# bruAristimunha/Synthetic-Sleep-EEG-Signal-Generation-using-Latent-Diffusion-Models

Measured on AMD Instinct MI355X. Metric: EEG windows/sec (LDM train step), higher is better.
Workload: dtype bf16; 1 GPU; LDM train step on raw (B,1,3072) windows: frozen AutoencoderKL[32,32,64] encode+sample x scale, add_noise, config_ldm.yaml UNet (30.5M params, latent_channels=1) fwd+bwd, epsilon MSE, Adam lr 1e-4 [BASELINE configs[2]/[3]: per-GPU batch 256 = global 2048 / 8]; per_gpu_batch=256, global_batch=256, latent_len=768, parallelism=dp1

## Files before the change

synthetic-sleep-eeg-signal-generation-using-latent-diffusion-models_amd/csrc/internal.h:

```cpp
#pragma once
#include "common.h"

int ew_temb(eegldm_ctx*, const int64_t* t, void* out, int B, int dim, int dtype);
int ew_silu(eegldm_ctx*, const float* x, void* y, long n, int dtype);
int ew_silu_bwd(eegldm_ctx*, const float* dy, const float* x, void* dx, long n, int dtype);
int eeg_det_buffer(eegldm_ctx*, size_t bytes, float** out);
int ew_fold_partials_det(eegldm_ctx*, const float* parts, int nparts, long stride, int off, int n, float* total);
int ew_colsum(eegldm_ctx*, const void* x, long ldx, float* out_ps, long ldo, float* total, int B, int L, int C, int dtype);
int ew_softmax(eegldm_ctx*, const float* S, void* P, long rows, int n, int dtype);
int ew_softmax_bwd(eegldm_ctx*, const float* dP, const void* P, void* dS, long rows, int n, float alpha, int dtype);
int ew_add_rows(eegldm_ctx*, void* dst, long ldd, const void* src, long lds, long rows, int C, int dtype);
int ew_dropout_rows(eegldm_ctx*, void* x, long ld, long rows, int C, float p, uint64_t seed, uint64_t offset, int dtype);
int ew_film_silu_fwd(eegldm_ctx*, const void* hn, long ldh, const float* emb, long lde, void* a, long lda, int B, int L, int C, int dtype);
int ew_film_silu_bwd(eegldm_ctx*, const void* hn, long ldh, const float* emb, long lde, const void* da, long ldda, void* dhn, long lddh,
                     float* demb, long ldde, int B, int L, int C, int dtype);
int ew_copy_rows(eegldm_ctx*, void* dst, long ldd, const void* src, long lds, long rows, int C, int dtype);
int ew_label_emb_add(eegldm_ctx*, float* emb, long ld, const int64_t* y, const float* table, int B, int te, int K);
int ew_label_emb_grad(eegldm_ctx*, const float* demb, long ld, const int64_t* y, int B, int te, int K, float* dtable);
int ew_label_dropout(eegldm_ctx*, const int64_t* y, int64_t* out, int B, float p, int64_t null_class, uint64_t seed, uint64_t offset);
int ew_emb_gather(eegldm_ctx*, const float* table, const int64_t* y, int K, int w, float* out, int B);

bool conv_is_thin(int Cin, int Cout, int dtype);
struct KbDesc { long off; long chunk0; int cout, cin; };
int kblk_pack(eegldm_ctx* ctx, const void* w_plain, void* w_packed, const KbDesc* d_table, int n, long total_chunks);
int kblk_pack_one(eegldm_ctx* ctx, const void* w_plain, void* w_packed, int Cout, int Cin, int taps = 3);
int kblk_pack_t(eegldm_ctx* ctx, const void* w_plain, void* w_packed, const KbDesc* d_table, int n, long total_chunks);
int kblk_pack_t_one(eegldm_ctx* ctx, const void* w_plain, void* w_packed, int Cout, int Cin, int taps = 3);
int s2ws_pack(eegldm_ctx* ctx, const void* w, void* wf, void* wd, int Cout, int Cin);
int dconv_run(eegldm_ctx*, int dtype, bool dgrad, const void* in, long ldin, const void* w, const float* bias,
              const void* resid, long ldr, void* out, long ldout, int B, int Lin, int Lout, int Cin, int Cout, int K,
              int stride, int pad_l, float act_slope = 0.f);
bool dconv_fuses_act(int dtype, int Cin, int Cout, int K, long ldout);
int dconv_wgrad(eegldm_ctx*, int dtype, const void* x, long ldx, const void* dy, long lddy, float* dw, int B, int Lin,
                int Lout, int Cin, int Cout, int K, int stride, int pad_l, float* dbias, int* bias_done);
bool dconv_wgrad_tinyv_ok(int Cin, int Cout, int K);

struct SkinnyGn { const float2* part; const float* gamma; const float* beta; int cpg; float eps; int silu;
                  const float2* part_b = nullptr; int nqa = 0; };
struct SkinnyExt { const void* x2; long ldx2; const void* w2; int Cin2; const float* bias2; };
bool conv_skinny_takes(int dtype, int Cin, int Cout, int taps, int B, int L);
int conv_skinny_ex(eegldm_ctx* ctx, int dtype, const void* x, long ldx, const void* w, int Cin, int Cout, int taps, const float* bias,
                   const float* rowvec, long ld_rowvec, const void* resid, long ldr, void* y, long ldy, int B, int L,
                   const SkinnyGn* gn, float2* part_out, const SkinnyExt* ext = nullptr);
int conv_skinny_try(eegldm_ctx* ctx, int dtype, const void* x, long ldx, const void* w, int Cin, int Cout, int taps, const float* bias,
                    const float* rowvec, long ld_rowvec, const void* resid, long ldr, void* y, long ldy, int B, int L);
int conv_ws2_try(eegldm_ctx*, int dtype, int dgrad, const void* x, const void* w, const float* bias, void* y, int B, int Lo,
                 float* col_parts = nullptr, int* col_nparts = nullptr);
int conv_ws_try(eegldm_ctx*, int dtype, const void* x, long ldx, const void* w, int Cin, int Cout, int transposed, const float* bias,
                const float* rowvec, long ld_rowvec, const void* resid, long ldr, void* y, long ldy, int B, int L,
                float* col_parts = nullptr, int* col_nparts = nullptr);

int op_conv_fwd(eegldm_ctx*, int dtype, const void* x, long ldx, const void* w, const float* bias, void* y, long ldy,
                int B, int Lin, int Cin, int Cout, int K, int stride, int pad_l, int pad_r,
                const float* rowvec, long ld_rowvec, const void* resid, long ldr, float act_slope = 0.f,
                float* col_parts = nullptr, int* col_nparts = nullptr);
bool op_conv_fuses_act(int dtype, int Cin, int Cout, int K, long ldy);
int op_conv3_skip_fwd(eegldm_ctx*, int dtype, const void* x, long ldx, const void* w, const float* bias, const void* x2, long ldx2,
                      const void* w2, const float* bias2, void* y, long ldy, int B, int L, int Cin, int Cin2, int Cout,
                      const float* rowvec, long ld_rowvec);
int op_conv_dgrad(eegldm_ctx*, int dtype, const void* dy, long lddy, const void* w, void* dx, long lddx,
                  int B, int Lin, int Cin, int Cout, int K, int stride, int pad_l, int pad_r, const void* resid, long ldr);
bool op_wgrad_fuses_bias(int dtype, int Cin, int Cout);
int op_gn_fold_flush(eegldm_ctx*);
int op_wgrad_flush(eegldm_ctx*);
int op_conv_wgrad(eegldm_ctx*, int dtype, const void* x, long ldx, const void* dy, long lddy, float* dw, float* dbias,
                  int B, int Lin, int Cin, int Cout, int K, int stride, int pad_l, int pad_r);
int op_linear(eegldm_ctx*, int dtype, const void* x, long ldx, const void* w, long ldw, const float* bias, void* y, long ldy,
              int M, int N, int K, int out_f32);
int op_linear_dgrad(eegldm_ctx*, int dtype, const void* dy, long lddy, const void* w, long ldw, void* dx, long lddx,
                    int M, int N, int K, int out_f32);
int op_linear_wgrad(eegldm_ctx*, int dtype, const void* x, long ldx, const void* dy, long lddy, float* dw, long lddw,
                    int M, int N, int K);
int op_attention_fwd(eegldm_ctx*, int dtype, const void* qkv, long ldq, void* out, long ldo, void* probs, float* logits,
                     int B, int T, int C);
int op_attention_bwd(eegldm_ctx*, int dtype, const void* qkv, long ldq, const void* probs, const void* dout, long lddo,
                     void* dqkv, long lddq, float* dprobs, void* dlogits, int B, int T, int C);
int op_groupnorm_bwd(eegldm_ctx*, const void* x, long ldx, const float* gamma, const float* beta, const float* stats,
                     const void* dy, long lddy, void* dx, long lddx, float* dgamma, float* dbeta, int B, int L, int C, int G,
                     int fuse_silu, int resample, const void* dxr, long lddxr, int dtype, float* colsum_ps, long ldps, int* colsum_done,
                     const void* dxr2 = nullptr, long lddxr2 = 0, int* dxr2_done = nullptr, int* slots_deferred = nullptr, int defer_region = 0);
int op_gn_slot_reduce_deferred(eegldm_ctx*, float* dgamma, float* dbeta, int C, int region = 0);
int ew_fold_partials(eegldm_ctx*, const float* parts, int nparts, int n, float* total);
bool pre_conv3_ok(int dtype, int Cin, int Cout, int L);
int pre_conv3_launch(eegldm_ctx*, const void* x, const double* in_stats, const float* gamma, const float* beta, const void* w,
                     const float* bias, const void* resid, void* y, double* out_stats, int B, int L, int Cin, int Cout, float eps, int dtype);
int sample_stats_launch(eegldm_ctx*, const void* x, long n_per_sample, int B, double* stats, int dtype);
bool attn_chain_ok(int dtype, int T, int C, long ldq, long ldo);
int attn_chain_fwd(eegldm_ctx*, const void* qkv, long ldq, void* out, long ldo, void* probs, int B, int T, int C, int dtype);
int attn_chain_bwd(eegldm_ctx*, const void* qkv, long ldq, const void* probs, const void* dout, long lddo, void* dq, long lddq,
                   void* dS, int B, int T, int C, int fuse_kv, int dtype);
bool attn_chain_bwd_fuses_kv(eegldm_ctx*, int B, int T);
```

synthetic-sleep-eeg-signal-generation-using-latent-diffusion-models_amd/csrc/ops.hip:

```cpp
#include <math.h>

#include "common.h"
#include "internal.h"
#include <string.h>

static inline int conv_lout(int Lin, int K, int stride, int pad_l, int pad_r) { return (Lin + pad_l + pad_r - K) / stride + 1; }

bool op_conv_fuses_act(int dtype, int Cin, int Cout, int K, long ldy) { return conv_is_thin(Cin, Cout, dtype) && dconv_fuses_act(dtype, Cin, Cout, K, ldy); }
int op_conv_fwd(eegldm_ctx* ctx, int dtype, const void* x, long ldx, const void* w, const float* bias, void* y, long ldy,
                int B, int Lin, int Cin, int Cout, int K, int stride, int pad_l, int pad_r,
                const float* rowvec, long ld_rowvec, const void* resid, long ldr, float act_slope, float* col_parts, int* col_nparts) {
  if (col_nparts) *col_nparts = 0;
  EEG_CHECK(B > 0 && Lin > 0 && Cin > 0 && Cout > 0 && (K == 1 || K == 3) && (stride == 1 || stride == 2),
            "unsupported conv B=%d Lin=%d Cin=%d Cout=%d K=%d stride=%d", B, Lin, Cin, Cout, K, stride);
  const int Lout = conv_lout(Lin, K, stride, pad_l, pad_r);
  EEG_CHECK(Lout > 0, "empty output");
  if (conv_is_thin(Cin, Cout, dtype)) {
    EEG_CHECK(rowvec == nullptr, "rowvec add is not available on the thin-channel path");
    return dconv_run(ctx, dtype, false, x, ldx, w, bias, resid, ldr, y, ldy, B, Lin, Lout, Cin, Cout, K, stride, pad_l, act_slope);
  }
  EEG_CHECK(act_slope <= 0.f, "fused activation is only available on the thin-input direct conv");
  if (K == 3 && stride == 2 && pad_l == 1 && pad_r == 1 && Cin == 64 && Cout == 128 && ldx == Cin && Lin == 2 * Lout && !rowvec && !resid &&
      dtype != EEGLDM_F32 && !ctx->s2ws_f.empty()) {
    auto it = ctx->s2ws_f.find(w);
// ... 105 lines not shown

int op_conv_wgrad(eegldm_ctx* ctx, int dtype, const void* x, long ldx, const void* dy, long lddy, float* dw, float* dbias,
                  int B, int Lin, int Cin, int Cout, int K, int stride, int pad_l, int pad_r) {
  const int Lout = conv_lout(Lin, K, stride, pad_l, pad_r);
  const bool thin = conv_is_thin(Cin, Cout, dtype);
  if (thin) {
    EEG_ENV_VAR(bool, fuse_bias, getenv("EEGLDM_NO_FUSED_BIAS_GRAD") == nullptr);
    int done = 0;
    EEG_TRY(dconv_wgrad(ctx, dtype, x, ldx, dy, lddy, dw, B, Lin, Lout, Cin, Cout, K, stride, pad_l, fuse_bias ? dbias : nullptr, &done));
    if (dbias && !done) EEG_TRY(ew_colsum(ctx, dy, lddy, nullptr, 0, dbias, B, Lout, Cout, dtype));
    return 0;
  }
  const bool bias_in_gemm = dbias && op_wgrad_fuses_bias(dtype, Cin, Cout);
  if (dbias && !bias_in_gemm) EEG_TRY(ew_colsum(ctx, dy, lddy, nullptr, 0, dbias, B, Lout, Cout, dtype));
  GemmArgs a = {};
  a.colsum = bias_in_gemm ? dbias : nullptr;
  a.dtype = dtype; a.amode = GA_TR; a.bmode = GB_TR;
  a.A = dy; a.lda = lddy; a.B = x; a.ldb = ldx; a.C = dw; a.ldc = Cin; a.sCt = (long)Cout * Cin;
  a.M = Cout; a.N = Cin; a.K = B * Lout; a.batch = 1; a.taps = 1; a.ztaps = K; a.alpha = 1.0f;
  a.conv_map = !(K == 1 && stride == 1 && pad_l == 0);
  a.Lout = Lout; a.Lin = Lin; a.stride = stride; a.pad_l = pad_l;
  a.out_f32 = 1; a.atomic_out = 1;
  const int kstage = 2 * (dtype == EEGLDM_F32 ? 16 : 32);
  const bool fused3 = (K == 3 && stride == 1 && pad_l == 1 && pad_r == 1 && Lout % kstage == 0);
  int bn = Cin > 64 ? 128 : (Cin > 32 ? 64 : 32);
  long tiles;
  int blocks_per_cu = 2;
  if (fused3) {
    a.taps = 3; a.ztaps = 1; a.conv_map = 0;
    bn = Cin > 32 ? 64 : 32;
    tiles = (long)((Cout + 127) / 128) * ((Cin + bn - 1) / bn);
  } else {
    tiles = (long)((Cout + 127) / 128) * ((Cin + bn - 1) / bn) * K;
  }
  long want = ((long)ctx->num_cu * blocks_per_cu) / tiles;
  long maxs = ((long)a.K + 8 * kstage - 1) / (8 * kstage);
  if (want > maxs) want = maxs;
  a.splitk = (int)(want < 1 ? 1 : want);
  if (ctx->defer_wgrad && (fused3 || (K == 1 && stride == 1 && pad_l == 0 && pad_r == 0)) && a.K % kstage == 0 && !a.wide_n &&
      a.M % 16 == 0 && a.N % 4 == 0) {
    WgradRec r; r.a = a; r.tiles = tiles; r.kstage = kstage; r.dst = dw; r.dbias = bias_in_gemm ? dbias : nullptr;
    r.a.colsum = nullptr; r.a.C = nullptr;
    ctx->wgrad_pending.push_back(r);
    return 0;
  }
  return gemm_launch(ctx, a);
}

int op_wgrad_flush(eegldm_ctx* ctx) {
  std::vector<WgradRec> recs; recs.swap(ctx->wgrad_pending);
  if (recs.empty()) return 0;
  std::vector<char> done(recs.size(), 0);
  const long slots = (long)ctx->num_cu * 2;
  for (size_t i = 0; i < recs.size(); i++) {
    if (done[i]) continue;
    const GemmArgs& k = recs[i].a;
    GemmArgs g = k; g.ngroup = 0;
    GemmGroup tab; memset(&tab, 0, sizeof(tab));
    for (size_t j = i; j < recs.size() && g.ngroup < GEMM_MAX_GROUP; j++) {
      const GemmArgs& o = recs[j].a;
      if (done[j] || o.dtype != k.dtype || o.taps != k.taps || o.ztaps != k.ztaps || o.M != k.M || o.N != k.N || o.K != k.K ||
          o.Lout != k.Lout || o.Lin != k.Lin || o.conv_map != k.conv_map || recs[j].tiles != recs[i].tiles) continue;
      tab.A[g.ngroup] = o.A; tab.B[g.ngroup] = o.B; tab.CS[g.ngroup] = recs[j].dbias; tab.Dst[g.ngroup] = recs[j].dst;
      tab.lda[g.ngroup] = o.lda; tab.ldb[g.ngroup] = o.ldb;
      g.ngroup++; done[j] = 1;
    }
    const long tiles_total = recs[i].tiles * g.ngroup, S = ((long)g.K + recs[i].kstage - 1) / recs[i].kstage;
    long maxs = S / 8; if (maxs < 1) maxs = 1; if (maxs > 256) maxs = 256;
    double best = 1e30; int bs = 1;
    constexpr double c_fixed = 8.0, c_block = 0.05;
    for (long sp = 1; sp <= maxs; sp++) {
      const long blocks = tiles_total * sp, rounds = (blocks + slots - 1) / slots;
      const double cost = (double)rounds * ((double)S / (double)sp + c_fixed) + c_block * (double)blocks;
      if (cost < best) { best = cost; bs = (int)sp; }
    }
    g.splitk = bs; g.batch = g.ngroup;
    EEG_TRY(gemm_launch_grouped(ctx, g, tab, ctx->grp_slot++));
  }
  return 0;
}

int op_linear(eegldm_ctx* ctx, int dtype, const void* x, long ldx, const void* w, long ldw, const float* bias, void* y, long ldy,
              int M, int N, int K, int out_f32) {
  GemmArgs a = {};
  a.dtype = dtype; a.amode = GA_PLAIN; a.bmode = GB_NT; a.A = x; a.lda = ldx; a.B = w; a.ldb = ldw; a.C = y; a.ldc = ldy;
  a.M = M; a.N = N; a.K = K; a.batch = 1; a.taps = 1; a.alpha = 1.0f; a.bias = bias; a.out_f32 = out_f32;
  return gemm_launch(ctx, a);
}
int op_linear_dgrad(eegldm_ctx* ctx, int dtype, const void* dy, long lddy, const void* w, long ldw, void* dx, long lddx,
                    int M, int N, int K, int out_f32) {
  GemmArgs a = {};
  a.dtype = dtype; a.amode = GA_PLAIN; a.bmode = GB_TR; a.A = dy; a.lda = lddy; a.B = w; a.ldb = ldw; a.C = dx; a.ldc = lddx;
  a.M = M; a.N = K; a.K = N; a.batch = 1; a.taps = 1; a.alpha = 1.0f; a.out_f32 = out_f32;
  const long tiles = (long)((M + 127) / 128) * ((K + 127) / 128);
  if (out_f32 && tiles * 8 < ctx->num_cu && N >= 1024) {
    long sk = ctx->num_cu / tiles; const long maxs = N / 256; if (sk > maxs) sk = maxs;
    if (sk > 1) {
      HIP_TRY(hipMemset2DAsync(dx, (size_t)lddx * 4, 0, (size_t)K * 4, M, ctx->stream));
      a.splitk = (int)sk;
    }
  }
  return gemm_launch(ctx, a);
}
int op_linear_wgrad(eegldm_ctx* ctx, int dtype, const void* x, long ldx, const void* dy, long lddy, float* dw, long lddw,
                    int M, int N, int K) {
  GemmArgs a = {};
  a.dtype = dtype; a.amode = GA_TR; a.bmode = GB_TR; a.A = dy; a.lda = lddy; a.B = x; a.ldb = ldx; a.C = dw; a.ldc = lddw;
  a.M = N; a.N = K; a.K = M; a.batch = 1; a.taps = 1; a.alpha = 1.0f; a.out_f32 = 1; a.atomic_out = 1;
  return gemm_launch(ctx, a);
}

int op_attention_fwd(eegldm_ctx* ctx, int dtype, const void* qkv, long ldq, void* out, long ldo, void* probs, float* logits,
                     int B, int T, int C) {
  if (attn_chain_ok(dtype, T, C, ldq, ldo)) return attn_chain_fwd(ctx, qkv, ldq, out, ldo, probs, B, T, C, dtype);
  const size_t es = dtype_size(dtype);
  const char* q = (const char*)qkv; const char* k = q + (size_t)C * es; const char* v = q + (size_t)2 * C * es;
  GemmArgs a = {};
  a.dtype = dtype; a.amode = GA_PLAIN; a.bmode = GB_NT; a.A = q; a.lda = ldq; a.sAb = (long)T * ldq; a.B = k; a.ldb = ldq;
  a.sBb = (long)T * ldq; a.C = logits; a.ldc = T; a.sCb = (long)T * T; a.M = T; a.N = T; a.K = C; a.batch = B; a.taps = 1;
  a.alpha = 1.0f / sqrtf((float)C);
  a.out_f32 = 1;
  EEG_TRY(gemm_launch(ctx, a));
  EEG_TRY(ew_softmax(ctx, logits, probs, (long)B * T, T, dtype));
  GemmArgs b = {};
  b.dtype = dtype; b.amode = GA_PLAIN; b.bmode = GB_TR; b.A = probs; b.lda = T; b.sAb = (long)T * T; b.B = v; b.ldb = ldq;
  b.sBb = (long)T * ldq; b.C = out; b.ldc = ldo; b.sCb = (long)T * ldo; b.M = T; b.N = C; b.K = T; b.batch = B; b.taps = 1;
  b.alpha = 1.0f;
  return gemm_launch(ctx, b);
}

int op_attention_bwd(eegldm_ctx* ctx, int dtype, const void* qkv, long ldq, const void* probs, const void* dout, long lddo,
                     void* dqkv, long lddq, float* dprobs, void* dlogits, int B, int T, int C) {
  const size_t es = dtype_size(dtype);
  const char* q = (const char*)qkv; const char* k = q + (size_t)C * es; const char* v = q + (size_t)2 * C * es;
  char* dq = (char*)dqkv; char* dk = dq + (size_t)C * es; char* dv = dq + (size_t)2 * C * es;
  const float alpha = 1.0f / sqrtf((float)C);
  GemmArgs g = {};
  const bool fused = attn_chain_ok(dtype, T, C, ldq, lddo) && lddq % 8 == 0;
  EEG_ENV_VAR(bool, no_fused_v, getenv("EEGLDM_ATTN_NO_FUSED_DV") != nullptr);
  const int fk = (fused && attn_chain_bwd_fuses_kv(ctx, B, T)) ? (no_fused_v ? 1 : 2) : 0;
  if (fk != 2) {
  g.dtype = dtype; g.amode = GA_TR; g.bmode = GB_TR; g.A = probs; g.lda = T; g.sAb = (long)T * T; g.B = dout; g.ldb = lddo;
  g.sBb = (long)T * lddo; g.C = dv; g.ldc = lddq; g.sCb = (long)T * lddq; g.M = T; g.N = C; g.K = T; g.batch = B; g.taps = 1; g.alpha = 1.f;
  EEG_TRY(gemm_launch(ctx, g));
  }
  if (fused) {
    EEG_TRY(attn_chain_bwd(ctx, qkv, ldq, probs, dout, lddo, dq, lddq, dlogits, B, T, C, fk, dtype));
    if (fk) return 0;
  } else {
  g = GemmArgs{};
  g.dtype = dtype; g.amode = GA_PLAIN; g.bmode = GB_NT; g.A = dout; g.lda = lddo; g.sAb = (long)T * lddo; g.B = v; g.ldb = ldq;
  g.sBb = (long)T * ldq; g.C = dprobs; g.ldc = T; g.sCb = (long)T * T; g.M = T; g.N = T; g.K = C; g.batch = B; g.taps = 1; g.alpha = 1.f;
  g.out_f32 = 1;
  EEG_TRY(gemm_launch(ctx, g));
  EEG_TRY(ew_softmax_bwd(ctx, dprobs, probs, dlogits, (long)B * T, T, alpha, dtype));
  g = GemmArgs{};
  g.dtype = dtype; g.amode = GA_PLAIN; g.bmode = GB_TR; g.A = dlogits; g.lda = T; g.sAb = (long)T * T; g.B = k; g.ldb = ldq;
  g.sBb = (long)T * ldq; g.C = dq; g.ldc = lddq; g.sCb = (long)T * lddq; g.M = T; g.N = C; g.K = T; g.batch = B; g.taps = 1; g.alpha = 1.f;
  EEG_TRY(gemm_launch(ctx, g));
  }
  g = GemmArgs{};
  g.dtype = dtype; g.amode = GA_TR; g.bmode = GB_TR; g.A = dlogits; g.lda = T; g.sAb = (long)T * T; g.B = q; g.ldb = ldq;
  g.sBb = (long)T * ldq; g.C = dk; g.ldc = lddq; g.sCb = (long)T * lddq; g.M = T; g.N = C; g.K = T; g.batch = B; g.taps = 1; g.alpha = 1.f;
  return gemm_launch(ctx, g);
}

extern "C" int eegldm_conv1d_fwd(eegldm_ctx* ctx, const void* x, long ldx, const void* w, const float* bias, void* y, long ldy,
                                 int B, int Lin, int Cin, int Cout, int K, int stride, int pad_l, int pad_r,
                                 const float* rowvec, long ld_rowvec, const void* resid, long ld_resid, int dtype) {
  EEG_CHECK(ctx && x && w && y, "null pointer");
  return op_conv_fwd(ctx, dtype, x, ldx, w, bias, y, ldy, B, Lin, Cin, Cout, K, stride, pad_l, pad_r, rowvec, ld_rowvec, resid, ld_resid);
}
extern "C" int eegldm_conv1d_pack_kblocked(eegldm_ctx* ctx, const void* w, void* w_kblocked, int Cout, int Cin, int dtype) {
  return eegldm_conv1d_pack_kblocked_k(ctx, w, w_kblocked, Cout, Cin, 3, dtype);
}
extern "C" int eegldm_conv1d_pack_kblocked_k(eegldm_ctx* ctx, const void* w, void* w_kblocked, int Cout, int Cin, int K, int dtype) {
  EEG_CHECK(K == 1 || K == 3, "kernel size 1 or 3");
  EEG_CHECK(ctx && w && w_kblocked && w != w_kblocked, "null or aliased pointer");
  EEG_CHECK(dtype != EEGLDM_F32 && Cin > 0 && Cout > 0 && Cin % 32 == 0, "K-blocked weights: 16-bit dtype and Cin %% 32 == 0 (got dtype %d, Cin %d)", dtype, Cin);
  EEG_CHECK(((size_t)w % 16 == 0) && ((size_t)w_kblocked % 16 == 0), "weights must be 16-byte aligned");
  EEG_TRY(kblk_pack_one(ctx, w, w_kblocked, Cout, Cin, K));
  ctx->kblk[w] = w_kblocked;
  return 0;
}
extern "C" int eegldm_conv1d_pack_dgrad(eegldm_ctx* ctx, const void* w, void* w_t, int Cout, int Cin, int dtype) {
  return eegldm_conv1d_pack_dgrad_k(ctx, w, w_t, Cout, Cin, 3, dtype);
}
extern "C" int eegldm_conv1d_pack_dgrad_k(eegldm_ctx* ctx, const void* w, void* w_t, int Cout, int Cin, int K, int dtype) {
// ... 92 lines not shown
```

synthetic-sleep-eeg-signal-generation-using-latent-diffusion-models_amd/csrc/unet.hip:

```cpp
#include <string.h>

#include <string>
#include <vector>

#include "net.h"

namespace {
constexpr int GN_G = 32;
struct Layer { int kind; ResDesc r; AttnDesc a; RsDesc s; };
inline int layer_cin(const Layer& l) { return l.kind == 0 ? l.r.cin : (l.kind == 1 ? l.a.c : l.s.c); }
inline int layer_cout(const Layer& l) { return l.kind == 0 ? l.r.cout : (l.kind == 1 ? l.a.c : l.s.c); }
inline int layer_len(const Layer& l, int L) {
  if (l.kind == 0) return l.r.updown == 1 ? L / 2 : (l.r.updown == 2 ? L * 2 : L);
  if (l.kind == 2) return l.s.up ? L * 2 : L / 2;
  return L;
}
struct Block { std::vector<Layer> layers; int cin, cout; };
}

struct eegldm_unet : NetBase {
  eegldm_unet_cfg cfg;
  int mc, te;
  long off_emb_w = 0, off_emb_b = 0, off_te0_w, off_te0_b, off_te2_w, off_te2_b, off_cin_w, off_cin_b, off_out_gw, off_out_gb, off_out_w, off_out_b;
  std::vector<Block> in_blocks, out_blocks; Block mid;
// ... 166 lines not shown
      ALLOC_OR_FAIL(dx.p, u->alloc_act(rows, cin)); dx.ld = cin; dx.C = cin;
    }
    int fused = 0;
    if (l.kind == 0) { EEG_TRY(res_backward(u, l.r, u->rt[--ri], dout, dx, demb_all, j == 0 ? extra : nullptr, &fused)); }
    else if (l.kind == 1) { EEG_TRY(attn_backward(u, l.a, u->at[--ai], dout, dx)); }
    else { const RsTape t = u->st.back(); u->st.pop_back(); EEG_TRY(resample_backward(u, l.s, t, dout, dx)); }
    if (j == 0 && extra && !fused) EEG_TRY(ew_add_rows(u->ctx, dx.p, dx.ld, extra->p, extra->ld, extra_rows, extra->C, u->dtype));
    dout = dx;
  }
  return 0;
}

}

static int unet_create(eegldm_ctx* ctx, const eegldm_unet_cfg* cfg, int num_classes, eegldm_unet** out) {
  EEG_CHECK(ctx && cfg && out, "null argument");
  EEG_CHECK(cfg->num_heads >= 0 && cfg->num_heads <= 64 && cfg->num_heads_upsample <= 64, "bad num_heads");
  {
    const int nh = cfg->num_heads > 0 ? cfg->num_heads : 1, nu = cfg->num_heads_upsample > 0 ? cfg->num_heads_upsample : nh;
    for (int i = 0; i < cfg->n_mult; i++) {
      const int chn = cfg->channel_mult[i] * cfg->model_channels;
      if (cfg->num_head_channels > 0) EEG_CHECK(chn % cfg->num_head_channels == 0 && cfg->num_head_channels % 8 == 0,
                                                "num_head_channels=%d must divide %d channels and be a multiple of 8", cfg->num_head_channels, chn);
      else EEG_CHECK(chn % nh == 0 && chn % nu == 0 && (chn / nh) % 8 == 0 && (chn / nu) % 8 == 0,
                     "%d channels / %d (%d) heads: the head width must be a whole multiple of 8", chn, nh, nu);
    }
  }
  EEG_CHECK(cfg->model_channels % 32 == 0, "model_channels must be a multiple of 32 (GroupNorm(32))");
  EEG_CHECK(cfg->n_mult >= 1 && cfg->n_mult <= 8 && cfg->n_attn >= 0 && cfg->n_attn <= 8, "bad channel_mult / attention_resolutions");
  EEG_CHECK(cfg->dtype == EEGLDM_F32 || cfg->dtype == EEGLDM_BF16 || cfg->dtype == EEGLDM_F16, "bad dtype");
  eegldm_unet* u = new eegldm_unet();
  u->ctx = ctx; u->cfg = *cfg; u->dtype = cfg->dtype; u->num_classes = num_classes;
  int rc = build_plan(u);
  if (rc) { delete u; return rc; }
  *out = u;
  return 0;
}
extern "C" int eegldm_unet_create(eegldm_ctx* ctx, const eegldm_unet_cfg* cfg, eegldm_unet** out) { return unet_create(ctx, cfg, 0, out); }
extern "C" int eegldm_unet_create_cond(eegldm_ctx* ctx, const eegldm_unet_cfg* cfg, int num_classes, eegldm_unet** out) {
  EEG_CHECK(num_classes >= 1 && num_classes <= (1 << 20), "num_classes=%d must be >= 1", num_classes);
  return unet_create(ctx, cfg, num_classes, out);
}
int unet_num_classes(const eegldm_unet* u) { return u->num_classes; }
eegldm_ctx* unet_ctx(const eegldm_unet* u) { return u->ctx; }
int unet_in_channels(const eegldm_unet* u) { return u->cfg.in_channels; }
int unet_out_channels(const eegldm_unet* u) { return u->cfg.out_channels; }
extern "C" int eegldm_unet_destroy(eegldm_unet* u) {
  if (!u) return 0;
  sampler_release(u);
  if (u->fuse_stats) (void)hipFree(u->fuse_stats);
  delete u;
  return 0;
}
extern "C" int eegldm_unet_set_dropout(eegldm_unet* u, float p, uint64_t seed) {
  EEG_CHECK(u, "null unet");
  EEG_CHECK(p >= 0.f && p < 1.f, "dropout probability %g outside [0, 1)", (double)p);
  u->dropout = p; u->drop_seed = seed; u->drop_ctr = 0;
  return 0;
}
extern "C" int eegldm_unet_num_entries(const eegldm_unet* u) { return (int)u->entries.size(); }
extern "C" long eegldm_unet_num_params(const eegldm_unet* u) { return u->nparams; }
extern "C" int eegldm_unet_set_grad_hook(eegldm_unet* u, eegldm_grad_hook fn, void* user) {
  EEG_CHECK(u, "null unet");
  u->grad_hook = fn; u->grad_hook_user = user;
  return 0;
}
extern "C" int eegldm_unet_entry(const eegldm_unet* u, int i, char* name, int cap, long* offset, long* numel, int* ndim, int shape[3]) {
  return entry_query(u, i, name, cap, offset, numel, ndim, shape);
}
extern "C" int eegldm_unet_bind(eegldm_unet* u, float* params, float* grads) {
  EEG_CHECK(u && params, "null argument");
  sampler_release(u);
  return u->bind(params, grads);
}
extern "C" int eegldm_unet_sync_weights(eegldm_unet* u) {
  EEG_CHECK(u, "null argument");
  return u->sync_weights();
}

static int embed_chain(eegldm_unet* u, const int64_t* tsteps, const int64_t* labels, int n, float* e0, float* h1e, float* a1e, float* emb,
                       float* semb, float* emb_all) {
  eegldm_ctx* ctx = u->ctx; const int mc = u->mc, te = u->te, F = EEGLDM_F32;
  EEG_TRY(ew_temb(ctx, tsteps, e0, n, mc, F));
  EEG_TRY(op_linear(ctx, F, e0, mc, u->P(u->off_te0_w), mc, u->P(u->off_te0_b), h1e, te, n, te, mc, 1));
  EEG_TRY(ew_silu(ctx, h1e, a1e, (long)n * te, F));
  EEG_TRY(op_linear(ctx, F, a1e, te, u->P(u->off_te2_w), te, u->P(u->off_te2_b), emb, te, n, te, te, 1));
  if (u->num_classes > 0) EEG_TRY(ew_label_emb_add(ctx, emb, te, labels, u->P(u->off_label), n, te, u->num_classes));
  EEG_TRY(ew_silu(ctx, emb, semb, (long)n * te, F));
  return op_linear(ctx, F, semb, te, u->P(u->off_emb_w), te, u->P(u->off_emb_b), emb_all, u->etot, n, u->etot, te, 1);
}
int unet_emb_width(const eegldm_unet* u) { return u->etot; }
long unet_embed_work_floats(const eegldm_unet* u) { return (long)u->mc + 4L * u->te; }
int unet_embed_table(eegldm_unet* u, const int64_t* tsteps_dev, const int64_t* labels_dev, int n, float* table, float* work) {
  EEG_CHECK(u && u->params && tsteps_dev && table && work && n > 0, "bad argument");
  EEG_CHECK(u->num_classes == 0 || labels_dev, "a class-conditional UNet's embedding rows need labels");
  const long te = u->te;
  float* e0 = work; float* h1e = e0 + (long)n * u->mc; float* a1e = h1e + n * te; float* emb = a1e + n * te; float* semb = emb + n * te;
  return embed_chain(u, tsteps_dev, labels_dev, n, e0, h1e, a1e, emb, semb, table);
}
void unet_set_shared_emb(eegldm_unet* u, const float* rows, long ld) { u->emb_shared = rows; u->emb_shared_ld = ld; }

struct LabelArg { const int64_t* y = nullptr; float p_uncond = 0.f; int64_t null_class = 0; uint64_t seed = 0, offset = 0; };
static int unet_forward_impl(eegldm_unet* u, const float* x, const int64_t* tsteps, const LabelArg& lab, float* y, int B, int L, int training) {
  EEG_CHECK(u && x && tsteps && y, "null argument");
  EEG_CHECK(u->params, "bind parameters first");
  EEG_CHECK(B > 0 && L > 0 && (L % (1 << (u->cfg.n_mult - 1))) == 0, "L=%d must be divisible by 2^(levels-1)", L);
  eegldm_ctx* ctx = u->ctx; const int dt = u->dtype; const int mc = u->mc, te = u->te;
  u->arena.reset(); u->rt.clear(); u->at.clear(); u->st.clear(); u->in_out.clear(); u->cat.clear();
  u->B = B; u->L = L; u->have_tape = false; u->training = training != 0;

  {
    EEG_ENV_VAR(bool, no_fuse, getenv("EEGLDM_NO_EVAL_GN_FUSE") != nullptr);
    u->eval_fuse = !training && !no_fuse && (dt == EEGLDM_BF16 || dt == EEGLDM_F16); u->fused_used = false; u->fuse_used = 0; u->part_reg.clear();
    if (u->eval_fuse) {
      size_t nres = 0; int cmax = 0;
      auto count = [&](const Block& b) { for (auto& l : b.layers) { nres++; if (l.kind == 0 && l.r.cout > cmax) cmax = l.r.cout; } };
      for (auto& b : u->in_blocks) count(b);
      count(u->mid);
      for (auto& b : u->out_blocks) count(b);
      const size_t need = 2 * nres * (size_t)B * (L / 16 + 1) * (cmax / 4);
      if (need > (size_t)4 << 20) u->eval_fuse = false;
      else if (u->fuse_cap < need) {
        HIP_TRY(hipStreamSynchronize(ctx->stream));
        if (u->fuse_stats) (void)hipFree(u->fuse_stats);
        u->fuse_stats = nullptr; u->fuse_cap = 0;
        HIP_TRY(hipMalloc(&u->fuse_stats, sizeof(float2) * need)); u->fuse_cap = need;
      }
    }
  }

  u->labels = nullptr;
  if (u->emb_shared && !training) {
    u->emb_all = const_cast<float*>(u->emb_shared); u->emb_ld = u->emb_shared_ld;
  } else {
    if (u->num_classes > 0) {
      EEG_CHECK(lab.y, "a class-conditional UNet needs labels");
      ALLOC_OR_FAIL(u->labels, (int64_t*)u->arena.alloc(sizeof(int64_t) * (size_t)B));
      EEG_TRY(ew_label_dropout(ctx, lab.y, u->labels, B, lab.p_uncond, lab.null_class, lab.seed, lab.offset));
    }
    auto fbuf = [&](long n) { return (float*)u->arena.alloc(sizeof(float) * (size_t)n); };
    ALLOC_OR_FAIL(u->e0, fbuf((long)B * mc));
    ALLOC_OR_FAIL(u->h1e, fbuf((long)B * te));
    ALLOC_OR_FAIL(u->a1e, fbuf((long)B * te));
    ALLOC_OR_FAIL(u->emb, fbuf((long)B * te));
    ALLOC_OR_FAIL(u->semb, fbuf((long)B * te));
    ALLOC_OR_FAIL(u->emb_all, fbuf((long)B * u->etot));
    u->emb_ld = u->etot;
    EEG_TRY(embed_chain(u, tsteps, u->labels, B, u->e0, u->h1e, u->a1e, u->emb, u->semb, u->emb_all));
  }

  const int n_in = (int)u->in_blocks.size(), n_out = (int)u->out_blocks.size();
  std::vector<int> in_len(n_in), in_ch(n_in);
  { int Lc = L; in_len[0] = L; in_ch[0] = mc;
    for (int i = 1; i < n_in; i++) { Lc = block_out_len(u->in_blocks[i], Lc); in_len[i] = Lc; in_ch[i] = u->in_blocks[i].cout; } }
  u->cat.resize(n_out);
  for (int j = 0; j < n_out; j++) {
    const int i = n_in - 1 - j, c1 = u->skip_c1[j], C = c1 + in_ch[i];
    ALLOC_OR_FAIL(u->cat[j].p, u->alloc_act((long)B * in_len[i], C)); u->cat[j].ld = C; u->cat[j].C = C;
  }
  u->in_out.resize(n_in);
  for (int i = 0; i < n_in; i++) { const int j = n_in - 1 - i; u->in_out[i] = col_view(u->cat[j], u->skip_c1[j], in_ch[i], dt); }

  ALLOC_OR_FAIL(u->x0.p, u->alloc_act((long)B * L, u->cfg.in_channels)); u->x0.ld = u->cfg.in_channels; u->x0.C = u->cfg.in_channels;
  EEG_TRY(eegldm_ncl_to_nlc(ctx, x, u->x0.p, u->x0.ld, B, u->cfg.in_channels, L, dt));
  EEG_TRY(op_conv_fwd(ctx, dt, u->x0.p, u->x0.ld, u->W(u->off_cin_w), u->P(u->off_cin_b), u->in_out[0].p, u->in_out[0].ld, B, L,
                      u->cfg.in_channels, mc, 3, 1, 1, 1, nullptr, 0, nullptr, 0));
  View h = u->in_out[0]; int Lc = L;
  for (int i = 1; i < n_in; i++) { EEG_TRY(block_forward(u, u->in_blocks[i], h, B, Lc, u->in_out[i])); h = u->in_out[i]; }
  { View dst = col_view(u->cat[0], 0, u->skip_c1[0], dt); EEG_TRY(block_forward(u, u->mid, h, B, Lc, dst)); }
  for (int j = 0; j < n_out; j++) {
    View dst;
// ... 179 lines not shown
```

synthetic-sleep-eeg-signal-generation-using-latent-diffusion-models_amd/sampling.py:

```python
import ctypes as C
import os

import numpy as np
import torch

from ._lib import lib, check, ptr, PRED
from .schedulers import DDIMScheduler, DPMSolverMultistepScheduler, RESAMPLE_KEY, scheduler_edit_tables, scheduler_resample_tables
from .training import randn


def _step_tables(scheduler):
    from .schedulers import DDPMScheduler
    ts = [int(t) for t in scheduler.timesteps]
    acp = scheduler.alphas_cumprod
    ancestral = isinstance(scheduler, DDPMScheduler)
    if ancestral:
        prev = [t - 1 for t in ts]
        final = 1.0
    else:
        ratio = scheduler.num_train_timesteps // scheduler.num_inference_steps
        prev = [t - ratio for t in ts]
        final = scheduler.final_alpha_cumprod
    a_t = [float(acp[t]) for t in ts]
    a_prev = [float(acp[p]) if p >= 0 else float(final) for p in prev]
# ... 170 lines not shown
    tail = (ptr(lat), ptr(win), B, L, 1 if use_graph else 0, C.byref(used))
    if edit is not None:
        z0, m_win, m_lat, init_d = _edit_inputs(unet, autoencoder, x, init, mask, init_latents,
                                                lambda w, native: _encode_windows(unet, autoencoder, w, scale_factor, native))
        nul = C.POINTER(C.c_float)()
        coef = (f32(tab["cx"]), f32(tab["c0"]), f32(tab["c1"])) if multistep else (nul, nul, nul)
        front = (unet.h, ae_h, ptr(x), ptr(z0), ptr(m_lat), i64(ts), f32(a_t), nul if multistep else f32(tab["a_prev"]), *coef,
                 f32(tab["a_next"]), n, PRED[scheduler.prediction_type], int(scheduler.clip_sample), 1.0 / float(scale_factor))
        back = (*tail, None if lab is None else i64(lab), float(guidance_scale), nc)
        if rt is None:
            check(lib.eegldm_sample_edit(*front, *back))
        else:
            check(lib.eegldm_sample_edit_resample(*front, f32(rt["jump_x"]), f32(rt["jump_n"]), RESAMPLE_KEY + int(seed), *back))
        if edit["composite"]:
            check(lib.eegldm_edit_window(unet.ctx.h, ptr(m_win), B, L * down, down, 0, None, ptr(init_d), ptr(win), out_c, ptr(win)))
    elif multistep:
        check(lib.eegldm_sample_multistep(unet.h, ae_h, ptr(x), i64(ts), f32(a_t), f32(cx), f32(c0), f32(c1), n, PRED[scheduler.prediction_type],
                                          int(scheduler.clip_sample), 1.0 / float(scale_factor), *tail, None if lab is None else i64(lab),
                                          float(guidance_scale), nc))
    else:
        args = (unet.h, ae_h, ptr(x), i64(ts), f32(a_t), f32(a_prev), f32(beta), n, 1 if ancestral else 0, PRED[scheduler.prediction_type],
                int(scheduler.clip_sample), 1.0 / float(scale_factor), int(seed), *tail)
        if lab is None:
            check(lib.eegldm_sample(*args))
        else:
            check(lib.eegldm_sample_cond(*args, i64(lab), float(guidance_scale), nc))
    unet._bump_tape()
    if autoencoder is not None:
        autoencoder._bump_tape()
    if info is not None:
        info["graph"], info["forwards"] = bool(used.value), n
    return (win[:, :, crop:-crop] if crop else win), lat


sample = ddim_sample


@torch.no_grad()
def ddim_sample_hostloop(unet, autoencoder, scheduler, noise, scale_factor=1.0, crop=36, labels=None, guidance_scale=1.0, null_class=None,
                         init=None, strength=1.0, mask=None, composite=None, init_latents=None, resamples=1, jump_length=1, seed=0):
    edit = _edit_args(autoencoder, scheduler, noise.shape, init, strength, mask, composite, init_latents)
    rt = _resample_args(scheduler, edit, mask, resamples, jump_length)
    unet.eval()
    x = noise.to(unet.device, torch.float32).contiguous()
    B = x.shape[0]
    lab, nc = _labels_host(unet, labels, B, guidance_scale, null_class)
    kw = {} if lab is None else {"y": torch.tensor(lab, dtype=torch.int64, device=unet.device)}
    null = None if lab is None else torch.full((B,), nc, dtype=torch.int64, device=unet.device)
    w = float(guidance_scale)
    tt = torch.empty(B, device=unet.device, dtype=torch.int64)
    timesteps, first = scheduler.timesteps, {}
    if edit is not None:
        tab = edit["tab"]
        nz = x
        z0, m_win, m_lat, init_d = _edit_inputs(unet, autoencoder, x, init, mask, init_latents,
                                                lambda w, native: _encode_windows(unet, autoencoder, w, scale_factor, native), native=False)
        x = _renoise(z0, nz, tab["a_t"][0])
        timesteps = tab["timesteps"]
        if isinstance(scheduler, DPMSolverMultistepScheduler):
            first = {"first_order": True}
        if rt is not None:
            tab, timesteps = rt, rt["timesteps"]
    jumps = 0
    for j, t in enumerate(timesteps):
        jumped = rt is not None and rt["jump_n"][j] != 0.0
        if jumped:
            x = _jump(unet.ctx, x, z0, nz, m_lat, rt, j, jumps, seed)
            jumps += 1
        tt.fill_(int(t))
        out = unet(x, timesteps=tt, **kw)
        if lab is not None and w != 1.0:
            out_u = unet(x, timesteps=tt, y=null)
            out = out_u + w * (out - out_u)
        x, _ = scheduler.step(out, int(t), x, **(first if j == 0 or jumped else {}))
        if edit is not None and m_lat is not None:
            x = m_lat * _renoise(z0, nz, tab["a_next"][j]) + (1.0 - m_lat) * x
    comp = (lambda win: m_win * init_d + (1.0 - m_win) * win) if edit is not None and edit["composite"] else (lambda win: win)
    if autoencoder is None:
        sample = comp(x)
        return (sample[:, :, crop:-crop] if crop else sample), x
    z = x
    if float(scale_factor) != 1.0:
        z = x.clone()
        alpha = 1.0 / float(scale_factor) - 1.0
        if edit is not None:
            alpha = float(np.float32(1.0 / float(scale_factor)) - np.float32(1.0))
        check(lib.eegldm_axpy(unet.ctx.h, ptr(z), ptr(z), alpha, z.numel()))
    sample = comp(autoencoder.decode_stage_2_outputs(z))
    return (sample[:, :, crop:-crop] if crop else sample), x


def make_sampling_scheduler(num_inference_steps=50, prediction_type="epsilon", beta_start=0.0015, beta_end=0.0205, device=0, sampler="ddim",
                            solver_order=2):
    if sampler == "dpmpp_2m":
        s = DPMSolverMultistepScheduler(num_train_timesteps=1000, schedule="scaled_linear_beta", beta_start=beta_start, beta_end=beta_end,
                                        prediction_type=prediction_type, clip_sample=False, solver_order=solver_order, device=device)
        s.set_timesteps(num_inference_steps)
        return s
    if sampler != "ddim":
        raise ValueError('sampler must be "ddim" or "dpmpp_2m"')
    s = DDIMScheduler(num_train_timesteps=1000, schedule="scaled_linear_beta", beta_start=beta_start, beta_end=beta_end,
                      prediction_type=prediction_type, clip_sample=False, device=device)
    s.set_timesteps(num_inference_steps)
    return s


def sample_seeds(unet, autoencoder, scheduler, seeds, latent_len=768, scale_factor=1.0, crop=36, labels=None, guidance_scale=1.0, null_class=None):
    lat = unet.in_channels
    noise = torch.empty(len(seeds), lat, latent_len, device=unet.device)
    for i, sd in enumerate(seeds):
        noise[i] = randn(unet.ctx, (lat, latent_len), seed=int(sd))
    return ddim_sample(unet, autoencoder, scheduler, noise, scale_factor, crop, labels=labels, guidance_scale=guidance_scale, null_class=null_class)


class LongLayout:

    def __init__(self, n_windows, window_len, margin, ramp):
        W, L, m, r = int(n_windows), int(window_len), int(margin), int(ramp)
        if (W, L, m, r) != (n_windows, window_len, margin, ramp):
            raise ValueError("n_windows, window_len, margin and ramp must be integers")
        if W < 1 or m < 0 or r < 0:
            raise ValueError(f"needs n_windows >= 1, margin >= 0 and ramp >= 0 (got {W}, {m}, {r})")
        if L < 1 or L < 3 * m + 2 * r:
            raise ValueError(f"window_len {L} < 3 * margin + 2 * ramp = {3 * m + 2 * r}: more than two windows would carry weight somewhere")
        self.n_windows, self.window_len, self.margin, self.ramp = W, L, m, r
        self.stride = L - (2 * m + r)
        self.canvas_len = (W - 1) * self.stride + L
        self.starts = [k * self.stride for k in range(W)]

    def weights(self, k):
        W, L, S, m, r = self.n_windows, self.window_len, self.stride, self.margin, self.ramp
        if not 0 <= k < W:
            raise IndexError(f"window {k} of {W}")
        w = np.ones(L, np.float32)
        u = ((np.arange(r, dtype=np.float64) + 0.5) / r).astype(np.float32) if r else np.zeros(0, np.float32)
        if k > 0:
            w[:m] = 0.0
            w[m:m + r] = u
        if k < W - 1:
            w[S + m:S + m + r] = np.float32(1.0) - u
            w[S + m + r:] = 0.0
        return w

    def scaled(self, down):
        d = int(down)
        if d < 1:
            raise ValueError("down must be >= 1")
        return LongLayout(self.n_windows, self.window_len * d, self.margin * d, self.ramp * d)

    def seams(self):
        return [(k * self.stride + self.margin, k * self.stride + self.margin + self.ramp) for k in range(1, self.n_windows)]

    def owner(self):
        p = np.arange(self.canvas_len)
        k1 = np.where(p < self.stride + self.margin, 0, np.minimum(self.n_windows - 1, (p - self.margin) // self.stride))
        return k1, p - k1 * self.stride


def long_layout(n_windows, window_len, margin, ramp):
    return LongLayout(n_windows, window_len, margin, ramp)


def window_labels_from_hypnogram(stages, layout, down=1, sfreq=100.0, epoch_seconds=30.0):
    stages = np.asarray(stages).reshape(-1)
    out = []
    for k in range(layout.n_windows):
        t = (k * layout.stride + layout.window_len / 2.0) * down / float(sfreq)
        e = int(t // float(epoch_seconds))
        if e >= len(stages):
# ... 226 lines not shown
```

Before: 14710 windows/s.

## Add small-M fp32 linear MFMA kernel with split-K and fused SiLU for time embedding

Adds a dedicated fp32 MFMA GEMM kernel for linear layers with M up to 1024, covering the forward, dgrad and wgrad forms. It uses a 4-wave K split inside the block with a shared-memory reduction, plus optional cross-block split-K through atomics. The time-embedding MLP now fuses bias and SiLU into the GEMM epilogue, removing the separate elementwise launches. The aim is to cut launch count and underutilisation of the generic GEMM on these tiny embedding linears, which are a small share of the step. A sampling scale-factor rounding change rides along.

```diff
diff --git a/synthetic-sleep-eeg-signal-generation-using-latent-diffusion-models_amd/csrc/internal.h b/synthetic-sleep-eeg-signal-generation-using-latent-diffusion-models_amd/csrc/internal.h
--- a/synthetic-sleep-eeg-signal-generation-using-latent-diffusion-models_amd/csrc/internal.h
+++ b/synthetic-sleep-eeg-signal-generation-using-latent-diffusion-models_amd/csrc/internal.h
@@ -71,6 +71,10 @@
                     int M, int N, int K, int out_f32);
 int op_linear_wgrad(eegldm_ctx*, int dtype, const void* x, long ldx, const void* dy, long lddy, float* dw, long lddw,
                     int M, int N, int K);
+enum { LS_NT = 0, LS_NN = 1, LS_TN = 2 };
+constexpr int LINEAR_SMALL_MAX_M = 1024;
+int linear_small_try(eegldm_ctx*, int form, int dtype, const void* p, long ldp, const void* q, long ldq, const float* bias, float* out,
+                     long ldo, int M, int N, int K, float* act = nullptr, long ldact = 0);
 int op_attention_fwd(eegldm_ctx*, int dtype, const void* qkv, long ldq, void* out, long ldo, void* probs, float* logits,
                      int B, int T, int C);
 int op_attention_bwd(eegldm_ctx*, int dtype, const void* qkv, long ldq, const void* probs, const void* dout, long lddo,
diff --git a/synthetic-sleep-eeg-signal-generation-using-latent-diffusion-models_amd/csrc/linear_small.hip b/synthetic-sleep-eeg-signal-generation-using-latent-diffusion-models_amd/csrc/linear_small.hip
--- /dev/null
+++ b/synthetic-sleep-eeg-signal-generation-using-latent-diffusion-models_amd/csrc/linear_small.hip
@@ -0,0 +1,215 @@
+#include "internal.h"
+
+namespace {
+
+enum { LS_STORE = 0, LS_ACCUM = 1, LS_ATOMIC = 2 };
+
+struct LsArgs {
+  const float* A; long lda;
+  const float* B; long ldb;
+  float* C; long ldc;
+  int M, N, K;
+  int kper;
+  const float* bias;
+  float* act; long ldact;
+  int epi;
+};
+
+template <int F> struct LsVec;
+template <> struct LsVec<1> { typedef float T; };
+template <> struct LsVec<2> { typedef eeg_f32x2 T; };
+template <> struct LsVec<4> { typedef f32x4 T; };
+template <int F> __device__ __forceinline__ float ls_elem(const typename LsVec<F>::T& t, int f) { return t[f]; }
+template <> __device__ __forceinline__ float ls_elem<1>(const float& t, int) { return t; }
+
+template <int L, int F> struct LsRaw {
+  typedef typename LsVec<L == 0 ? 4 : F>::T V;
+  static constexpr int NV = L == 0 ? F : 4;
+  V t[NV]; bool in[NV];
+};
+template <int L, int F>
+__device__ __forceinline__ void ls_issue(LsRaw<L, F>& raw, const float* __restrict__ P, long ld, int x0, int X, int K, int kb, int kend, int lane) {
+  typedef typename LsRaw<L, F>::V V;
+  const int r = lane & 15, q = lane >> 4;
+  if constexpr (L == 0) {
+    const int k = kb + 4 * q;
+    const bool kin = k < kend;
+    const int kc = k < K - 4 ? k : K - 4;
+#pragma unroll
+    for (int f = 0; f < F; f++) {
+      const int x = x0 + 16 * f + r;
+      const int xc = x < X ? x : X - 1;
+      raw.t[f] = *(const V*)(P + (long)xc * ld + kc);
+      raw.in[f] = kin && x < X;
+    }
+  } else {
+    const int x = x0 + F * r;
+    const int xc = x < X ? x : X - F;
+#pragma unroll
+    for (int j = 0; j < 4; j++) {
+      const int k = kb + 4 * q + j;
+      const int kc = k < K ? k : K - 1;
+      raw.t[j] = *(const V*)(P + (long)kc * ld + xc);
+      raw.in[j] = k < kend && x < X;
+    }
+  }
+}
+template <int L, int F>
+__device__ __forceinline__ void ls_take(float (&v)[F][4], const LsRaw<L, F>& raw) {
+#pragma unroll
+  for (int f = 0; f < F; f++)
+#pragma unroll
+    for (int j = 0; j < 4; j++) {
+      if constexpr (L == 0) v[f][j] = raw.in[f] ? raw.t[f][j] : 0.f;
+      else v[f][j] = raw.in[j] ? ls_elem<F>(raw.t[j], f) : 0.f;
+    }
+}
+
+template <int LA, int LB, int FM, int FN>
+__global__ __launch_bounds__(256, (FM * FN >= 4 ? 4 : 8)) void linear_small_kernel(const LsArgs a) {
+  constexpr int BM = 16 * FM, BN = 16 * FN, LDR = BN + 4;
+  __shared__ __attribute__((aligned(16))) float red[4 * BM * LDR];
+  const int lane = threadIdx.x & 63, w = __builtin_amdgcn_readfirstlane(threadIdx.x >> 6);
+  const int m0 = blockIdx.y * BM, n0 = blockIdx.x * BN;
+  const int kz0 = blockIdx.z * a.kper, kz1 = kz0 + a.kper < a.K ? kz0 + a.kper : a.K;
+  const int per = (((kz1 - kz0 + 3) >> 2) + 15) & ~15;
+  const int k0 = kz0 + w * per, k1 = k0 + per < kz1 ? k0 + per : kz1;
+
+  f32x4 acc[FM][FN];
+#pragma unroll
+  for (int i = 0; i < FM; i++)
+#pragma unroll
+    for (int j = 0; j < FN; j++) acc[i][j] = f32x4{0.f, 0.f, 0.f, 0.f};
+
+  if (k0 < k1) {
+    float av[FM][4], bv[FN][4];
+    LsRaw<LA, FM> ra; LsRaw<LB, FN> rb;
+    ls_issue<LA, FM>(ra, a.A, a.lda, m0, a.M, a.K, k0, k1, lane);
+    ls_issue<LB, FN>(rb, a.B, a.ldb, n0, a.N, a.K, k0, k1, lane);
+    ls_take<LA, FM>(av, ra); ls_take<LB, FN>(bv, rb);
+    for (int kb = k0; kb < k1; kb += 16) {
+      ls_issue<LA, FM>(ra, a.A, a.lda, m0, a.M, a.K, kb + 16, k1, lane);
+      ls_issue<LB, FN>(rb, a.B, a.ldb, n0, a.N, a.K, kb + 16, k1, lane);
+      __builtin_amdgcn_sched_barrier(0);
+#pragma unroll
+      for (int j = 0; j < 4; j++)
+#pragma unroll
+        for (int fm = 0; fm < FM; fm++)
+#pragma unroll
+          for (int fn = 0; fn < FN; fn++) acc[fm][fn] = __builtin_amdgcn_mfma_f32_16x16x4f32(av[fm][j], bv[fn][j], acc[fm][fn], 0, 0, 0);
+      __builtin_amdgcn_sched_barrier(0);
+      ls_take<LA, FM>(av, ra); ls_take<LB, FN>(bv, rb);
+    }
+  }
+
+  {
+    float* R = red + w * (BM * LDR);
+    const int c = lane & 15, g = lane >> 4;
+#pragma unroll
+    for (int fm = 0; fm < FM; fm++)
+#pragma unroll
+      for (int fn = 0; fn < FN; fn++)
+#pragma unroll
+        for (int i = 0; i < 4; i++) {
+          const int row = LA ? FM * (4 * g + i) + fm : 16 * fm + 4 * g + i;
+          const int col = LB ? FN * c + fn : 16 * fn + c;
+          R[row * LDR + col] = acc[fm][fn][i];
+        }
+  }
+  __syncthreads();
+  for (int idx = threadIdx.x; idx < BM * (BN / 4); idx += 256) {
+    const int row = idx / (BN / 4), c4 = (idx % (BN / 4)) * 4;
+    const int m = m0 + row, n = n0 + c4;
+    if (m >= a.M || n >= a.N) continue;
+    float s[4];
+    {
+      const f32x4 t = *(const f32x4*)(red + row * LDR + c4);
+#pragma unroll
+      for (int j = 0; j < 4; j++) s[j] = t[j];
+    }
+#pragma unroll
+    for (int p = 1; p < 4; p++) {
+      const f32x4 t = *(const f32x4*)(red + p * (BM * LDR) + row * LDR + c4);
+#pragma unroll
+      for (int j = 0; j < 4; j++) s[j] += t[j];
+    }
+    float* dst = a.C + (long)m * a.ldc + n;
+    if (a.epi == LS_ATOMIC) {
+#pragma unroll
+      for (int j = 0; j < 4; j++) atomicAdd(dst + j, s[j]);
+      continue;
+    }
+    if (a.epi == LS_ACCUM) {
+      const f32x4 t = *(const f32x4*)dst;
+#pragma unroll
+      for (int j = 0; j < 4; j++) s[j] = t[j] + s[j];
+    } else if (a.bias) {
+      const f32x4 t = *(const f32x4*)(a.bias + n);
+#pragma unroll
+      for (int j = 0; j < 4; j++) s[j] += t[j];
+    }
+    *(f32x4*)dst = f32x4{s[0], s[1], s[2], s[3]};
+    if (a.act) *(f32x4*)(a.act + (long)m * a.ldact + n) = f32x4{silu_f(s[0]), silu_f(s[1]), silu_f(s[2]), silu_f(s[3])};
+  }
+}
+
+template <int LA, int LB, int FM, int FN>
+void ls_launch(eegldm_ctx* ctx, const LsArgs& a, int splitk) {
+  const dim3 grid((unsigned)((a.N + 16 * FN - 1) / (16 * FN)), (unsigned)((a.M + 16 * FM - 1) / (16 * FM)), (unsigned)splitk);
+  hipLaunchKernelGGL((linear_small_kernel<LA, LB, FM, FN>), grid, dim3(256), 0, ctx->stream, a);
+}
+
+inline bool al16(const void* p) { return ((uintptr_t)p & 15) == 0; }
+inline long cdiv(long a, long b) { return (a + b - 1) / b; }
+
+}
+
+bool linear_small_takes(int dtype, int form, int M, int N, int K, long lda, long ldb, long ldc) {
+  EEG_ENV_VAR(bool, off, getenv("EEGLDM_NO_LINEAR_SMALL") != nullptr && atoi(getenv("EEGLDM_NO_LINEAR_SMALL")) != 0);
+  if (off || dtype != EEGLDM_F32 || M < 1 || N < 1 || K < 1 || M > LINEAR_SMALL_MAX_M) return false;
+  if (N % 4 || K % 4 || lda % 4 || ldb % 4 || ldc % 4) return false;
+  (void)form;
+  return true;
+}
+
+int linear_small_try(eegldm_ctx* ctx, int form, int dtype, const void* p, long ldp, const void* q, long ldq, const float* bias, float* out,
+                     long ldo, int M, int N, int K, float* act, long ldact) {
+  if (!linear_small_takes(dtype, form, M, N, K, ldp, ldq, ldo)) return 0;
+  if (!al16(p) || !al16(q) || !al16(out) || (bias && !al16(bias)) || (act && (!al16(act) || ldact % 4))) return 0;
+  LsArgs a = {};
+  int cls;
+  if (form == LS_NT) { a.A = (const float*)p; a.lda = ldp; a.B = (const float*)q; a.ldb = ldq; a.M = M; a.N = N; a.K = K; a.epi = LS_STORE; cls = PROF_GEMM_NT; }
+  else if (form == LS_NN) { a.A = (const float*)p; a.lda = ldp; a.B = (const float*)q; a.ldb = ldq; a.M = M; a.N = K; a.K = N; a.epi = LS_STORE; cls = PROF_GEMM_NN; }
+  else { a.A = (const float*)q; a.lda = ldq; a.B = (const float*)p; a.ldb = ldp; a.M = N; a.N = K; a.K = M; a.epi = LS_ACCUM; cls = PROF_GEMM_TN; }
+  a.C = out; a.ldc = ldo; a.bias = bias; a.act = act; a.ldact = ldact;
+  const long tiles_big = cdiv(a.M, 32) * cdiv(a.N, 64);
+  const long tiles_small = cdiv(a.M, 16) * cdiv(a.N, 32);
+  auto slices = [&](long tiles) -> int {
+    if (form != LS_NN || a.K < 1024 || eeg_deterministic()) return 1;
+    long s = cdiv(2L * ctx->num_cu, tiles); const long maxs = a.K / 256;
+    if (s > maxs) s = maxs;
+    return s < 1 ? 1 : (int)s;
+  };
+  int splitk = slices(tiles_big);
+  const bool big = tiles_big * splitk >= ctx->num_cu;
+  if (!big) splitk = slices(tiles_small);
+  a.kper = (int)(cdiv(cdiv(a.K, splitk), 64) * 64);
+  splitk = (int)cdiv(a.K, a.kper);
+  ProfRec rec; const bool prof = ctx->prof_on;
+  if (prof) {
+    rec.cls = cls; rec.flops = 2.0 * a.M * a.N * (double)a.K; rec.M = a.M; rec.N = a.N; rec.K = a.K; rec.taps = 1; rec.splitk = splitk;
+    rec.kern = "linear_small";
+    HIP_TRY(hipEventCreate(&rec.a)); HIP_TRY(hipEventCreate(&rec.b));
+    HIP_TRY(hipEventRecord(rec.a, ctx->stream));
+  }
+  if (splitk > 1) {
+    HIP_TRY(hipMemset2DAsync(a.C, (size_t)a.ldc * 4, 0, (size_t)a.N * 4, a.M, ctx->stream));
+    a.epi = LS_ATOMIC;
+  }
+  if (form == LS_NT) { if (big) ls_launch<0, 0, 2, 4>(ctx, a, splitk); else ls_launch<0, 0, 1, 2>(ctx, a, splitk); }
+  else if (form == LS_NN) { if (big) ls_launch<0, 1, 2, 4>(ctx, a, splitk); else ls_launch<0, 1, 1, 2>(ctx, a, splitk); }
+  else { if (big) ls_launch<1, 1, 2, 4>(ctx, a, splitk); else ls_launch<1, 1, 1, 2>(ctx, a, splitk); }
+  LAUNCH_CHECK();
+  if (prof) { HIP_TRY(hipEventRecord(rec.b, ctx->stream)); ctx->prof.push_back(rec); }
+  return 1;
+}
diff --git a/synthetic-sleep-eeg-signal-generation-using-latent-diffusion-models_amd/csrc/ops.hip b/synthetic-sleep-eeg-signal-generation-using-latent-diffusion-models_amd/csrc/ops.hip
--- a/synthetic-sleep-eeg-signal-generation-using-latent-diffusion-models_amd/csrc/ops.hip
+++ b/synthetic-sleep-eeg-signal-generation-using-latent-diffusion-models_amd/csrc/ops.hip
@@ -211,6 +211,7 @@
 
 int op_linear(eegldm_ctx* ctx, int dtype, const void* x, long ldx, const void* w, long ldw, const float* bias, void* y, long ldy,
               int M, int N, int K, int out_f32) {
+  if (const int r = linear_small_try(ctx, LS_NT, dtype, x, ldx, w, ldw, bias, (float*)y, ldy, M, N, K)) return r < 0 ? r : 0;
   GemmArgs a = {};
   a.dtype = dtype; a.amode = GA_PLAIN; a.bmode = GB_NT; a.A = x; a.lda = ldx; a.B = w; a.ldb = ldw; a.C = y; a.ldc = ldy;
   a.M = M; a.N = N; a.K = K; a.batch = 1; a.taps = 1; a.alpha = 1.0f; a.bias = bias; a.out_f32 = out_f32;
@@ -218,6 +219,7 @@
 }
 int op_linear_dgrad(eegldm_ctx* ctx, int dtype, const void* dy, long lddy, const void* w, long ldw, void* dx, long lddx,
                     int M, int N, int K, int out_f32) {
+  if (const int r = linear_small_try(ctx, LS_NN, dtype, dy, lddy, w, ldw, nullptr, (float*)dx, lddx, M, N, K)) return r < 0 ? r : 0;
   GemmArgs a = {};
   a.dtype = dtype; a.amode = GA_PLAIN; a.bmode = GB_TR; a.A = dy; a.lda = lddy; a.B = w; a.ldb = ldw; a.C = dx; a.ldc = lddx;
   a.M = M; a.N = K; a.K = N; a.batch = 1; a.taps = 1; a.alpha = 1.0f; a.out_f32 = out_f32;
@@ -233,6 +235,7 @@
 }
 int op_linear_wgrad(eegldm_ctx* ctx, int dtype, const void* x, long ldx, const void* dy, long lddy, float* dw, long lddw,
                     int M, int N, int K) {
+  if (const int r = linear_small_try(ctx, LS_TN, dtype, x, ldx, dy, lddy, nullptr, dw, lddw, M, N, K)) return r < 0 ? r : 0;
   GemmArgs a = {};
   a.dtype = dtype; a.amode = GA_TR; a.bmode = GB_TR; a.A = dy; a.lda = lddy; a.B = x; a.ldb = ldx; a.C = dw; a.ldc = lddw;
   a.M = N; a.N = K; a.K = M; a.batch = 1; a.taps = 1; a.alpha = 1.0f; a.out_f32 = 1; a.atomic_out = 1;
diff --git a/synthetic-sleep-eeg-signal-generation-using-latent-diffusion-models_amd/csrc/unet.hip b/synthetic-sleep-eeg-signal-generation-using-latent-diffusion-models_amd/csrc/unet.hip
--- a/synthetic-sleep-eeg-signal-generation-using-latent-diffusion-models_amd/csrc/unet.hip
+++ b/synthetic-sleep-eeg-signal-generation-using-latent-diffusion-models_amd/csrc/unet.hip
@@ -272,11 +272,20 @@
                        float* semb, float* emb_all) {
   eegldm_ctx* ctx = u->ctx; const int mc = u->mc, te = u->te, F = EEGLDM_F32;
   EEG_TRY(ew_temb(ctx, tsteps, e0, n, mc, F));
-  EEG_TRY(op_linear(ctx, F, e0, mc, u->P(u->off_te0_w), mc, u->P(u->off_te0_b), h1e, te, n, te, mc, 1));
-  EEG_TRY(ew_silu(ctx, h1e, a1e, (long)n * te, F));
-  EEG_TRY(op_linear(ctx, F, a1e, te, u->P(u->off_te2_w), te, u->P(u->off_te2_b), emb, te, n, te, te, 1));
-  if (u->num_classes > 0) EEG_TRY(ew_label_emb_add(ctx, emb, te, labels, u->P(u->off_label), n, te, u->num_classes));
-  EEG_TRY(ew_silu(ctx, emb, semb, (long)n * te, F));
+  EEG_ENV_VAR(bool, nofuse, getenv("EEGLDM_LINEAR_SMALL_NO_FUSE") != nullptr && atoi(getenv("EEGLDM_LINEAR_SMALL_NO_FUSE")) != 0);
+  int fused = nofuse ? 0 : linear_small_try(ctx, LS_NT, F, e0, mc, u->P(u->off_te0_w), mc, u->P(u->off_te0_b), h1e, te, n, te, mc, a1e, te);
+  if (fused < 0) return fused;
+  if (!fused) {
+    EEG_TRY(op_linear(ctx, F, e0, mc, u->P(u->off_te0_w), mc, u->P(u->off_te0_b), h1e, te, n, te, mc, 1));
+    EEG_TRY(ew_silu(ctx, h1e, a1e, (long)n * te, F));
+  }
+  fused = (nofuse || u->num_classes > 0) ? 0 : linear_small_try(ctx, LS_NT, F, a1e, te, u->P(u->off_te2_w), te, u->P(u->off_te2_b), emb, te, n, te, te, semb, te);
+  if (fused < 0) return fused;
+  if (!fused) {
+    EEG_TRY(op_linear(ctx, F, a1e, te, u->P(u->off_te2_w), te, u->P(u->off_te2_b), emb, te, n, te, te, 1));
+    if (u->num_classes > 0) EEG_TRY(ew_label_emb_add(ctx, emb, te, labels, u->P(u->off_label), n, te, u->num_classes));
+    EEG_TRY(ew_silu(ctx, emb, semb, (long)n * te, F));
+  }
   return op_linear(ctx, F, semb, te, u->P(u->off_emb_w), te, u->P(u->off_emb_b), emb_all, u->etot, n, u->etot, te, 1);
 }
 int unet_emb_width(const eegldm_unet* u) { return u->etot; }
diff --git a/synthetic-sleep-eeg-signal-generation-using-latent-diffusion-models_amd/sampling.py b/synthetic-sleep-eeg-signal-generation-using-latent-diffusion-models_amd/sampling.py
--- a/synthetic-sleep-eeg-signal-generation-using-latent-diffusion-models_amd/sampling.py
+++ b/synthetic-sleep-eeg-signal-generation-using-latent-diffusion-models_amd/sampling.py
@@ -276,9 +276,7 @@
     z = x
     if float(scale_factor) != 1.0:
         z = x.clone()
-        alpha = 1.0 / float(scale_factor) - 1.0
-        if edit is not None:
-            alpha = float(np.float32(1.0 / float(scale_factor)) - np.float32(1.0))
+        alpha = float(np.float32(1.0 / float(scale_factor)) - np.float32(1.0))
         check(lib.eegldm_axpy(unet.ctx.h, ptr(z), ptr(z), alpha, z.numel()))
     sample = comp(autoencoder.decode_stage_2_outputs(z))
     return (sample[:, :, crop:-crop] if crop else sample), x
```

New measurement: 14840 windows/s, median of 6. No clear change (+0.9%).
